# microsoft/AI2BMD

Hardware: NVIDIA H100
Metric: MD steps/sec (higher is better)
Workload: dtype f32

## Files before the change

ai2bmd_b200/csrc/k_edge_tc.cuh:

```cuda
#pragma once
#include "k_edge.cuh"
#include "tc_common.cuh"

namespace vb {

constexpr int TC_TE = 128;
constexpr int TC_STAGES = 2;
constexpr int TC_MAX_STAGES = 3;
constexpr int TC_SLABS = D / tc::SLAB_K;
static_assert((TC_SLABS & (TC_SLABS - 1)) == 0, "tc_slab rotates the slab order with a mask: TC_SLABS must be a power of two");
constexpr int TC_MAXJOBS = 12;
constexpr int TC_LT = D + LDS_PAD;

struct TcJob {
    const float* img;
    int accumulate;
};

struct TcShared {
    alignas(1024) uint8_t ring[TC_STAGES][tc::STAGE_BYTES];
    alignas(16) float tile[TC_TE][TC_LT];
    alignas(16) float abuf[TC_TE][TC_LT];
    EdgeMeta<TC_TE> meta;
    alignas(8) uint64_t b_full[TC_MAX_STAGES];
    uint64_t b_tile;
    uint32_t released[TC_MAX_STAGES];
    const TcJob* jobs;
// ... 77 lines not shown
    __syncwarp();
    if (lane == 0) {
        const uint32_t before = tc::atom_add_acq_rel(&sh.released[k % NS], 1u);
        if (before % TC2_CWARPS == TC2_CWARPS - 1) tc_issue<NS>(sh, k + NS);
    }
}

__device__ __forceinline__ void tc2_tile_to_a(TcShared& sh, int rows) {
    csync();
    for (int idx = threadIdx.x; idx < rows * (D / 4); idx += TC2_CTHREADS) {
        const int r = idx >> 5, c = (idx & 31) * 4;
        st4(&sh.abuf[r][c], ld4(&sh.tile[r][c]));
    }
}

template <int ROWS>
__device__ __forceinline__ void tc2_mma(TcShared& sh, TcRing<ROWS>& ring, float (&acc)[32], int accumulate, int warp, int lane,
                                        int nvalid) {
    constexpr int NS = TcRing<ROWS>::NS;
    csync();
    const int q = warp >> 2, m0 = (q & 1) * 64 + (warp & 3) * 16, g = lane >> 2, t = lane & 3;
    const bool active = (q & 1) * 64 < nvalid;
    if (!accumulate) {
#pragma unroll
        for (int i = 0; i < 32; i++) acc[i] = 0.f;
    }
#pragma unroll 1
    for (int s = 0; s < TC_SLABS; s++) {
        const int k = ring.next + s, stage = k % NS;
        if (active) {
            uint32_t ahi[4][4], alo[4][4];
            const int k0 = tc_slab(s) * tc::SLAB_K + t;
#pragma unroll
            for (int kk = 0; kk < 4; kk++) {
                const int kc = k0 + kk * 8;
                tc::split_tf32(sh.abuf[m0 + g][kc], ahi[kk][0], alo[kk][0]);
                tc::split_tf32(sh.abuf[m0 + g + 8][kc], ahi[kk][1], alo[kk][1]);
                tc::split_tf32(sh.abuf[m0 + g][kc + 4], ahi[kk][2], alo[kk][2]);
                tc::split_tf32(sh.abuf[m0 + g + 8][kc + 4], ahi[kk][3], alo[kk][3]);
            }
            tc::mbar_wait(&sh.b_full[stage], (uint32_t)(k / NS) & 1u);
            const uint32_t bhi = tc::smem_u32(tc_stage_ptr(sh, stage)) + (uint32_t)(q >> 1) * (64 * 128);
            const uint32_t blo = bhi + tc::SLAB_BYTES;
            tc::wgmma_fence();
#pragma unroll
            for (int kk = 0; kk < 4; kk++) {
                const uint64_t dhi = tc::smem_desc_sw128(bhi + kk * 32);
                const uint64_t dlo = tc::smem_desc_sw128(blo + kk * 32);
                tc::mma_m64n64k8_tf32(acc, alo[kk], dhi);
                tc::mma_m64n64k8_tf32(acc, ahi[kk], dlo);
                tc::mma_m64n64k8_tf32(acc, ahi[kk], dhi);
            }
            tc::wgmma_commit();
            tc::wgmma_wait_all();
#pragma unroll
            for (int kk = 0; kk < 4; kk++)
#pragma unroll
                for (int i = 0; i < 4; i++) { tc::reg_fence(ahi[kk][i]); tc::reg_fence(alo[kk][i]); }
#pragma unroll
            for (int i = 0; i < 32; i++) tc::reg_fence(acc[i]);
        } else {
            tc::mbar_wait(&sh.b_full[stage], (uint32_t)(k / NS) & 1u);
        }
        tc2_release<NS>(sh, k, lane);
    }
    ring.next += TC_SLABS;
}

__device__ __forceinline__ void tc2_acc_to_tile(TcShared& sh, const float (&acc)[32], int warp, int lane, int nvalid) {
    const int q = warp >> 2, r = (q & 1) * 64 + (warp & 3) * 16 + (lane >> 2), c = (q >> 1) * 64 + 2 * (lane & 3);
#pragma unroll
    for (int i = 0; i < 8; i++) {
        if (r < nvalid) *reinterpret_cast<float2*>(&sh.tile[r][c + 8 * i]) = make_float2(acc[4 * i], acc[4 * i + 1]);
        if (r + 8 < nvalid) *reinterpret_cast<float2*>(&sh.tile[r + 8][c + 8 * i]) = make_float2(acc[4 * i + 2], acc[4 * i + 3]);
    }
}

template <int ROWS>
__global__ void __launch_bounds__(TC2_THREADS, 1) tc_selftest_kernel(const float* __restrict__ A, const float* __restrict__ img,
                                                                     float* __restrict__ Dout, int reps) {
    extern __shared__ __align__(1024) uint8_t dyn_raw[];
    TcShared& sh = *tc_shared_base(dyn_raw);
    __shared__ TcJob jobs[1];
    if (threadIdx.x == 0) jobs[0] = TcJob{img, 0};
    TcRing<ROWS> ring;
    tc2_setup(sh, ring, jobs, 1, reps);
    const int warp = threadIdx.x >> 5, lane = threadIdx.x & 31;
    float acc[32];
    for (int t = 0; t < reps; t++) {
        for (int idx = threadIdx.x; idx < ROWS * (D / 4); idx += TC2_CTHREADS) {
            const int r = idx >> 5, c = (idx & 31) * 4;
            st4(&sh.tile[r][c], ld4(A + (size_t)r * D + c));
        }
        tc2_tile_to_a(sh, ROWS);
        tc2_mma(sh, ring, acc, 0, warp, lane, ROWS);
        csync();
        tc2_acc_to_tile(sh, acc, warp, lane, ROWS);
        csync();
        for (int idx = threadIdx.x; idx < ROWS * (D / 4); idx += TC2_CTHREADS) {
            const int r = idx >> 5, c = (idx & 31) * 4;
            st4(Dout + (size_t)r * D + c, ld4(&sh.tile[r][c]));
        }
        csync();
    }
}

template <int ROWS>
__global__ void __launch_bounds__(TC2_THREADS, 1) edge_fwd_tc_kernel(const __grid_constant__ EdgeTcArgs a) {
    pdl_entry();
    extern __shared__ __align__(1024) uint8_t dyn_raw[];
    TcShared& sh = *tc_shared_base(dyn_raw);
    const Workspace& ws = a.ws;
    const int l = a.layer;
    const LayerW& lw = a.mw.layer[l];
    const bool upd = (l < L - 1);
    const int J_DK = 0, J_DV = 1, J_F = 2, J_S1 = upd ? 3 : 2, J_S2 = upd ? 4 : 3;
    constexpr int RPW = ROWS / TC2_CWARPS;
    const int warp = threadIdx.x >> 5, lane = threadIdx.x & 31, col = lane * 4;
    const int E = ws.rowptr[ws.N];
    const int trows = min(ROWS, max(16, a.tile_rows));
    const int ntiles_total = (E + trows - 1) / trows;
    const int my_tiles = ((int)blockIdx.x < ntiles_total) ? (ntiles_total - (int)blockIdx.x + (int)gridDim.x - 1) / (int)gridDim.x : 0;
    if (a.tl != nullptr && blockIdx.x == 0 && threadIdx.x == 0) a.tl[0] = (unsigned long long)clock64();
    TcRing<ROWS> ring;
    tc2_setup(sh, ring, a.jobs, a.njobs, my_tiles);
    if (a.tl != nullptr && blockIdx.x == 0 && threadIdx.x == 0) a.tl[1] = (unsigned long long)clock64();

    float acc[32];
    const float* __restrict__ Fin = ws.F[l];
    float* __restrict__ Fout = upd ? ws.F[l + 1] : nullptr;
    const float* __restrict__ QKV = ws.QKV[l];
    const float* __restrict__ VN = ws.VN[l];
// ... 10 lines not shown
        {
            constexpr int RW = ROWS / TC2_CWARPS;
            const int w0 = warp * RW, wn = max(0, min(RW, nvalid - w0));
            if (lane == 0) {
                if (wn > 0) tc::mbar_arrive_expect_tx(&sh.b_tile, (uint32_t)wn * D * 4);
                else tc::mbar_arrive(&sh.b_tile);
            }
            __syncwarp();
            if (lane < wn) tc::tma_load_1d(&sh.abuf[w0 + lane][0], Fin + (size_t)(e0 + w0 + lane) * D, D * 4, &sh.b_tile);
        }
        load_edge_meta<TC_TE, TC2_CTHREADS>(sh.meta, ws, e0, nvalid);
        tc::mbar_wait(&sh.b_tile, tpar);
        csync();
        TC_TL(2);
        float Areg[RPW];
        tc2_mma(sh, ring, acc, a.jobs[J_DK].accumulate, warp, lane, nvalid);
        TC_TL(4);
        tc2_acc_to_tile(sh, acc, warp, lane, nvalid);
        csync();
        {
            TC_TL(5);
            const float4 bb = ldg4(lw.b1 + col);
#pragma unroll
            for (int r = 0; r < RPW; r++) {
                if (r >= rpw) break;
                const int row = r0 + r;
                const float4 qi = ldg4(QKV + (size_t)sh.meta.dst[row] * 3 * D + col);
                const float4 kj = ldg4(QKV + (size_t)sh.meta.src[row] * 3 * D + D + col);
                const float4 P = ld4(&sh.tile[row][col]) + bb;
                const float av = quad_sum(hsum4(qi * kj * silu4(P)));
                Areg[r] = silu_(av) * sh.meta.C[row];
                if ((r < rpw && row < nvalid)) {
                    st4(P1 + (size_t)(e0 + row) * 3 * D + col, P);
                    if ((lane & 3) == 0) ATT[(size_t)(e0 + row) * H + (lane >> 2)] = av;
                }
            }
        }
        TC_TL(6);
        tc2_mma(sh, ring, acc, a.jobs[J_DV].accumulate, warp, lane, nvalid);
        TC_TL(7);
        csync();
        tc2_acc_to_tile(sh, acc, warp, lane, nvalid);
        csync();
        {
            TC_TL(8);
            const float4 bb = ldg4(lw.b1 + D + col);
#pragma unroll
            for (int r = 0; r < RPW; r++) {
                if (r >= rpw) break;
                const int row = r0 + r;
                const float4 vj = ldg4(QKV + (size_t)sh.meta.src[row] * 3 * D + 2 * D + col);
                const float4 P = ld4(&sh.tile[row][col]) + bb;
                st4(&sh.tile[row][col], vj * silu4(P) * Areg[r]);
                if ((r < rpw && row < nvalid)) st4(P1 + (size_t)(e0 + row) * 3 * D + D + col, P);
            }
        }
        csync();
        TC_TL(9);
        {
            const int i_first = sh.meta.dst[0], i_last = sh.meta.dst[nvalid - 1];
            for (int i = i_first + grp; i <= i_last; i += TC2_NGRP) {
                const int q0 = ws.rowptr[i], q1 = ws.rowptr[i + 1];
                const int lo = max(q0, e0) - e0, hi = min(q1, e0 + nvalid) - e0;
                float xa = 0.f;
                for (int r = lo; r < hi; r++) xa += sh.tile[r][cch];
                if (q0 >= e0 && q1 <= e0 + nvalid) ws.XA[(size_t)i * D + cch] = xa;
                else atomicAdd(ws.XA + (size_t)i * D + cch, xa);
            }
        }
        TC_TL(10);
        if (upd) tc2_mma(sh, ring, acc, a.jobs[J_F].accumulate, warp, lane, nvalid);
        tc2_tile_to_a(sh, nvalid);
        TC_TL(11);
        if (upd) {
            csync();
            tc2_acc_to_tile(sh, acc, warp, lane, nvalid);
            csync();
            const float4 bb = ldg4(lw.b1 + 2 * D + col);
#pragma unroll 1
            for (int rb = 0; rb < RPW; rb += 2) {
                if (rb >= rpw) break;
                float4 tir[2][3], ujr[2][3], fin[2];
#pragma unroll
                for (int u = 0; u < 2; u++) {
                    const int row = r0 + rb + u;
                    const size_t i3 = (size_t)sh.meta.dst[row] * 3, j3 = (size_t)sh.meta.src[row] * 3;
                    fin[u] = (rb + u < rpw && row < nvalid) ? ldg4(Fin + (size_t)(e0 + row) * D + col) : f4s(0.f);
#pragma unroll
                    for (int s = 0; s < 3; s++) {
                        tir[u][s] = ldg4(TU + (i3 + s) * 2 * D + col);
                        ujr[u][s] = ldg4(TU + (j3 + s) * 2 * D + D + col);
                    }
                }
#pragma unroll
                for (int u = 0; u < 2; u++) {
                    const int row = r0 + rb + u;
                    const float4 dd = sh.meta.d[row];
                    const float4 Pf = ld4(&sh.tile[row][col]) + bb;
                    const float4 fp = silu4(Pf);
                    const float4 a1 = tir[u][0] * dd.x + tir[u][1] * dd.y + tir[u][2] * dd.z;
                    const float4 a2 = ujr[u][0] * dd.x + ujr[u][1] * dd.y + ujr[u][2] * dd.z;
                    const float4 wdot = (tir[u][0] - a1 * dd.x) * (ujr[u][0] - a2 * dd.x) + (tir[u][1] - a1 * dd.y) * (ujr[u][1] - a2 * dd.y) +
                                        (tir[u][2] - a1 * dd.z) * (ujr[u][2] - a2 * dd.z);
                    if ((rb + u < rpw && row < nvalid)) {
                        st4(P1 + (size_t)(e0 + row) * 3 * D + 2 * D + col, Pf);
                        st4(Fout + (size_t)(e0 + row) * D + col, fin[u] + fp * wdot);
                    }
                }
            }
        }
        TC_TL(12);
        float bnd[2][3] = {{0.f, 0.f, 0.f}, {0.f, 0.f, 0.f}};
        tc2_mma(sh, ring, acc, a.jobs[J_S1].accumulate, warp, lane, nvalid);
        TC_TL(13);
        csync();
        tc2_acc_to_tile(sh, acc, warp, lane, nvalid);
        csync();
        {
            TC_TL(14);
            const float b = __ldg(lw.bs + cch);
            const int i_first = sh.meta.dst[0], i_last = sh.meta.dst[nvalid - 1];
            int nb = 0;
            for (int i = i_first + grp; i <= i_last; i += TC2_NGRP) {
                const int q0 = ws.rowptr[i], q1 = ws.rowptr[i + 1];
                const int lo = max(q0, e0) - e0, hi = min(q1, e0 + nvalid) - e0;
                float v0 = 0.f, v1 = 0.f, v2 = 0.f;
                int r = lo;
                for (; r + 4 <= hi; r += 4) {
                    float g[4][3], s1[4];
#pragma unroll
                    for (int u = 0; u < 4; u++) {
                        const size_t j3 = (size_t)sh.meta.src[r + u] * 3;
                        g[u][0] = __ldg(VN + (j3 + 0) * D + cch); g[u][1] = __ldg(VN + (j3 + 1) * D + cch); g[u][2] = __ldg(VN + (j3 + 2) * D + cch);
                        const float sp = sh.tile[r + u][cch] + b;
                        SP[(size_t)(e0 + r + u) * 2 * D + cch] = sp;
                        s1[u] = silu_(sp);
                    }
#pragma unroll
                    for (int u = 0; u < 4; u++) { v0 += g[u][0] * s1[u]; v1 += g[u][1] * s1[u]; v2 += g[u][2] * s1[u]; }
                }
                for (; r < hi; r++) {
                    const size_t j3 = (size_t)sh.meta.src[r] * 3;
                    const float sp = sh.tile[r][cch] + b;
                    SP[(size_t)(e0 + r) * 2 * D + cch] = sp;
                    const float s1 = silu_(sp);
                    v0 += __ldg(VN + (j3 + 0) * D + cch) * s1;
                    v1 += __ldg(VN + (j3 + 1) * D + cch) * s1;
                    v2 += __ldg(VN + (j3 + 2) * D + cch) * s1;
                }
                if (q0 >= e0 && q1 <= e0 + nvalid) {
                    ws.VA[((size_t)i * 3 + 0) * D + cch] = v0;
                    ws.VA[((size_t)i * 3 + 1) * D + cch] = v1;
                    ws.VA[((size_t)i * 3 + 2) * D + cch] = v2;
                } else if (nb < 2) {
                    bnd[nb][0] = v0; bnd[nb][1] = v1; bnd[nb][2] = v2;
                    nb++;
                }
            }
        }
        TC_TL(15);
        if (threadIdx.x == 0 && it + 1 < my_tiles) {
            const int en = ((int)blockIdx.x + (it + 1) * (int)gridDim.x) * trows;
            tc::tma_prefetch_l2(Fin + (size_t)en * D, (uint32_t)min(trows, E - en) * D * 4);
        }
        tc2_mma(sh, ring, acc, a.jobs[J_S2].accumulate, warp, lane, nvalid);
        TC_TL(16);
        csync();
        tc2_acc_to_tile(sh, acc, warp, lane, nvalid);
        csync();
        {
            TC_TL(17);
            const float b = __ldg(lw.bs + D + cch);
            const int i_first = sh.meta.dst[0], i_last = sh.meta.dst[nvalid - 1];
            int nb = 0;
            for (int i = i_first + grp; i <= i_last; i += TC2_NGRP) {
                const int q0 = ws.rowptr[i], q1 = ws.rowptr[i + 1];
                const int lo = max(q0, e0) - e0, hi = min(q1, e0 + nvalid) - e0;
                float v0 = 0.f, v1 = 0.f, v2 = 0.f;
                for (int r = lo; r < hi; r++) {
                    const float4 de = sh.meta.d[r];
                    const float sp = sh.tile[r][cch] + b;
                    SP[(size_t)(e0 + r) * 2 * D + D + cch] = sp;
                    const float s2 = silu_(sp);
                    v0 += s2 * de.x; v1 += s2 * de.y; v2 += s2 * de.z;
                }
                if (q0 >= e0 && q1 <= e0 + nvalid) {
                    ws.VA[((size_t)i * 3 + 0) * D + cch] += v0;
                    ws.VA[((size_t)i * 3 + 1) * D + cch] += v1;
                    ws.VA[((size_t)i * 3 + 2) * D + cch] += v2;
                } else if (nb < 2) {
                    atomicAdd(ws.VA + ((size_t)i * 3 + 0) * D + cch, bnd[nb][0] + v0);
                    atomicAdd(ws.VA + ((size_t)i * 3 + 1) * D + cch, bnd[nb][1] + v1);
                    atomicAdd(ws.VA + ((size_t)i * 3 + 2) * D + cch, bnd[nb][2] + v2);
                    nb++;
                }
            }
// ... 8 lines not shown

namespace vb {

template <int ROWS>
__global__ void __launch_bounds__(TC2_THREADS, 1) edge_bwd_tc_kernel(const __grid_constant__ EdgeTcArgs a) {
    pdl_entry();
    extern __shared__ __align__(1024) uint8_t dyn_raw[];
    TcShared& sh = *tc_shared_base(dyn_raw);
    const Workspace& ws = a.ws;
    const int l = a.layer;
    const bool upd = (l < L - 1);
    const int J_G3A = 0, J_G3B = 1, J_G4DV = 2, J_G4DK = 3, J_G4F = 4;
    const int J_LAST = upd ? J_G4F : J_G4DK;
    constexpr int RPW = ROWS / TC2_CWARPS;
    constexpr int RB4 = (RPW % 4 == 0) ? 4 : 2;
    const int warp = threadIdx.x >> 5, lane = threadIdx.x & 31, col = lane * 4, hd = lane >> 2;
    const int E = ws.rowptr[ws.N];
    const int trows = min(ROWS, max(16, a.tile_rows));
    const int ntiles_total = (E + trows - 1) / trows;
    const int my_tiles = ((int)blockIdx.x < ntiles_total) ? (ntiles_total - (int)blockIdx.x + (int)gridDim.x - 1) / (int)gridDim.x : 0;
    if (a.tl != nullptr && blockIdx.x == 0 && threadIdx.x == 0) a.tl[0] = (unsigned long long)clock64();
    TcRing<ROWS> ring;
    tc2_setup(sh, ring, a.jobs, a.njobs, my_tiles);
    if (a.tl != nullptr && blockIdx.x == 0 && threadIdx.x == 0) a.tl[1] = (unsigned long long)clock64();

    float acc[32];
    const float* __restrict__ QKV = ws.QKV[l];
    const float* __restrict__ VN = ws.VN[l];
    const float* __restrict__ TU = ws.TU[l];
    const float* __restrict__ P1 = ws.P1[l];
    const float* __restrict__ SP = ws.SP[l];
    const float* __restrict__ ATT = ws.ATT[l];
    const int cch = threadIdx.x & (D - 1), grp = threadIdx.x >> 7;
    for (int it = 0; it < my_tiles; it++) {
        const int e0 = ((int)blockIdx.x + it * (int)gridDim.x) * trows;
        const int nvalid = min(trows, E - e0);
        const int rpw = (nvalid + TC2_CWARPS - 1) / TC2_CWARPS, r0 = warp * rpw;
        load_edge_meta<TC_TE, TC2_CTHREADS>(sh.meta, ws, e0, nvalid);
        csync();
        TC_TL(2);
#pragma unroll 1
        for (int rb = 0; rb < RPW; rb += RB4) {
            if (rb >= rpw) break;
            float4 sp[RB4], gM[RB4][3], vn[RB4][3];
#pragma unroll
            for (int u = 0; u < RB4; u++) {
                const int row = r0 + rb + u;
                const size_t e = (size_t)(e0 + ((rb + u < rpw && row < nvalid) ? row : 0));
                const size_t i3 = (size_t)sh.meta.dst[row] * 3, j3 = (size_t)sh.meta.src[row] * 3;
                sp[u] = ldg4(SP + e * 2 * D + col);
#pragma unroll
                for (int s = 0; s < 3; s++) { gM[u][s] = ldg4(ws.GVEC + (i3 + s) * D + col); vn[u][s] = ldg4(VN + (j3 + s) * D + col); }
            }
#pragma unroll
            for (int u = 0; u < RB4; u++) {
                const int row = r0 + rb + u;
                const bool ok = (rb + u < rpw && row < nvalid);
                const size_t j3 = (size_t)sh.meta.src[row] * 3;
                const float4 s1 = silu4(sp[u]);
                const float4 gs1 = gM[u][0] * vn[u][0] + gM[u][1] * vn[u][1] + gM[u][2] * vn[u][2];
                if (rb + u < rpw) st4(&sh.abuf[row][col], ok ? gs1 * dsilu4(sp[u]) : f4s(0.f));
                if (ok) {
                    red4(ws.GVNMSG + (j3 + 0) * D + col, gM[u][0] * s1);
                    red4(ws.GVNMSG + (j3 + 1) * D + col, gM[u][1] * s1);
                    red4(ws.GVNMSG + (j3 + 2) * D + col, gM[u][2] * s1);
                }
            }
        }
        TC_TL(3);
#pragma unroll 4
        for (int r = 0; r < RPW; r++) {
            if (r >= rpw) break;
            const int row = r0 + r;
            const bool ok = (r < rpw && row < nvalid);
            const size_t e = (size_t)(e0 + (ok ? row : 0));
            const size_t i3 = (size_t)sh.meta.dst[row] * 3;
            const float4 dd = sh.meta.d[row];
            const float4 sp = ldg4(SP + e * 2 * D + D + col);
            const float4 s2 = silu4(sp);
            const float4 gM0 = ldg4(ws.GVEC + (i3 + 0) * D + col), gM1 = ldg4(ws.GVEC + (i3 + 1) * D + col),
                         gM2 = ldg4(ws.GVEC + (i3 + 2) * D + col);
            const float gx_ = warp_sum(hsum4(gM0 * s2)), gy_ = warp_sum(hsum4(gM1 * s2)), gz_ = warp_sum(hsum4(gM2 * s2));
            if (lane == 0) { sh.eacc[row][1] = gx_; sh.eacc[row][2] = gy_; sh.eacc[row][3] = gz_; }
            st4(&sh.tile[row][col], ok ? (gM0 * dd.x + gM1 * dd.y + gM2 * dd.z) * dsilu4(sp) : f4s(0.f));
        }
        TC_TL(5);
        csync();
        tc2_mma(sh, ring, acc, a.jobs[J_G3A].accumulate, warp, lane, nvalid);
        TC_TL(6);
        tc2_tile_to_a(sh, nvalid);
        TC_TL(7);
        tc2_mma(sh, ring, acc, a.jobs[J_G3B].accumulate, warp, lane, nvalid);
        TC_TL(8);
        csync();
        tc2_acc_to_tile(sh, acc, warp, lane, nvalid);
        csync();
        TC_TL(9);
#pragma unroll 1
        for (int rb = 0; rb < RPW; rb += RB4) {
            if (rb >= rpw) break;
            float4 gxa[RB4], vjr[RB4], pdvr[RB4];
            float avr[RB4];
#pragma unroll
            for (int u = 0; u < RB4; u++) {
                const int row = r0 + rb + u;
                const size_t e = (size_t)(e0 + ((rb + u < rpw && row < nvalid) ? row : 0));
                gxa[u] = load_gxa(ws, (size_t)sh.meta.dst[row], col);
                vjr[u] = ldg4(QKV + (size_t)sh.meta.src[row] * 3 * D + 2 * D + col);
                pdvr[u] = ldg4(P1 + e * 3 * D + D + col);
                avr[u] = (rb + u < rpw && row < nvalid) ? __ldg(ATT + e * H + hd) : 0.f;
            }
#pragma unroll
            for (int u = 0; u < RB4; u++) {
                const int row = r0 + rb + u;
                const bool ok = (rb + u < rpw && row < nvalid);
                const size_t j = sh.meta.src[row];
                const float Ce = sh.meta.C[row];
                const float av = avr[u], sa = silu_(av), A = sa * Ce;
                const bool mine = rb + u < rpw;
                const float4 gm = mine ? ld4(&sh.tile[row][col]) + gxa[u] : f4s(0.f);
                const float4 dv = silu4(pdvr[u]);
                if (mine) st4(&sh.abuf[row][col], ok ? gm * vjr[u] * A * dsilu4(pdvr[u]) : f4s(0.f));
                const float gA = quad_sum(hsum4(gm * vjr[u] * dv));
                if (mine && (lane & 3) == 0) sh.gattn[row][hd] = gA * Ce * dsilu_(av);
                const float gc = warp_sum((lane & 3) == 0 ? gA * sa : 0.f);
                if (mine && lane == 0) sh.eacc[row][0] = gc;
                if (ok) red4(ws.GQKV + j * 3 * D + 2 * D + col, gm * dv * A);
            }
// ... 8 lines not shown
            for (int u = 0; u < RB4; u++) {
                const int row = r0 + rb + u;
                const size_t e = (size_t)(e0 + ((rb + u < rpw && row < nvalid) ? row : 0));
                pdkr[u] = ldg4(P1 + e * 3 * D + col);
                qir[u] = ldg4(QKV + (size_t)sh.meta.dst[row] * 3 * D + col);
                kjr[u] = ldg4(QKV + (size_t)sh.meta.src[row] * 3 * D + D + col);
            }
#pragma unroll
            for (int u = 0; u < RB4; u++) {
                const int row = r0 + rb + u;
                const bool ok = (rb + u < rpw && row < nvalid);
                const size_t j = sh.meta.src[row];
                const float4 dk = silu4(pdkr[u]);
                const float gav = sh.gattn[row][hd];
                if (rb + u < rpw) st4(&sh.tile[row][col], ok ? qir[u] * kjr[u] * gav * dsilu4(pdkr[u]) : f4s(0.f));
                if (ok) red4(ws.GQKV + j * 3 * D + D + col, qir[u] * dk * gav);
            }
        }
        TC_TL(12);
        csync();
        tc2_mma(sh, ring, acc, a.jobs[J_G4DV].accumulate, warp, lane, nvalid);
        TC_TL(13);
        tc2_tile_to_a(sh, nvalid);
        TC_TL(14);
        csync();
#pragma unroll 4
        for (int r = 0; r < RPW; r++) {
            if (r >= rpw) break;
            const int row = r0 + r;
            const size_t e = (size_t)(e0 + ((r < rpw && row < nvalid) ? row : 0));
            const float4 dk = silu4(ldg4(P1 + e * 3 * D + col));
            const float4 kj = ldg4(QKV + (size_t)sh.meta.src[row] * 3 * D + D + col);
            st4(&sh.tile[row][col], kj * dk * sh.gattn[row][hd]);
        }
        csync();
        {
            const int i_first = sh.meta.dst[0], i_last = sh.meta.dst[nvalid - 1];
            for (int i = i_first + grp; i <= i_last; i += TC2_NGRP) {
                const int q0 = ws.rowptr[i], q1 = ws.rowptr[i + 1];
                const int lo = max(q0, e0) - e0, hi = min(q1, e0 + nvalid) - e0;
                float gq = 0.f;
                for (int r = lo; r < hi; r++) gq += sh.tile[r][cch];
                if (q0 >= e0 && q1 <= e0 + nvalid) ws.GQKV[(size_t)i * 3 * D + cch] = gq;
                else atomicAdd(ws.GQKV + (size_t)i * 3 * D + cch, gq);
            }
        }
        TC_TL(15);
        if (upd) {
            csync();
#pragma unroll 1
            for (int rb = 0; rb < RPW; rb += 2) {
                if (rb >= rpw) break;
                float4 gfr[2], pfr[2], tir[2][3], ujr[2][3];
#pragma unroll
                for (int u = 0; u < 2; u++) {
                    const int row = r0 + rb + u;
                    const bool ok = (rb + u < rpw && row < nvalid);
                    const size_t e = (size_t)(e0 + (ok ? row : 0));
                    const size_t i3 = (size_t)sh.meta.dst[row] * 3, j3 = (size_t)sh.meta.src[row] * 3;
                    gfr[u] = ok ? ld4(ws.GF + e * D + col) : f4s(0.f);
                    pfr[u] = ldg4(P1 + e * 3 * D + 2 * D + col);
#pragma unroll
                    for (int s = 0; s < 3; s++) {
// ... 6 lines not shown
                    const int row = r0 + rb + u;
                    const bool ok = (rb + u < rpw && row < nvalid);
                    const size_t e = (size_t)(e0 + (ok ? row : 0));
                    const size_t j3 = (size_t)sh.meta.src[row] * 3;
                    const float4 dd = sh.meta.d[row];
                    const float4 gfn = gfr[u], pf = pfr[u];
                    const float4 fp = silu4(pf);
                    const float dv3[3] = {dd.x, dd.y, dd.z};
                    const float4 a1 = tir[u][0] * dd.x + tir[u][1] * dd.y + tir[u][2] * dd.z;
                    const float4 a2 = ujr[u][0] * dd.x + ujr[u][1] * dd.y + ujr[u][2] * dd.z;
                    float4 w1[3], w2[3];
#pragma unroll
                    for (int s = 0; s < 3; s++) { w1[s] = tir[u][s] - a1 * dv3[s]; w2[s] = ujr[u][s] - a2 * dv3[s]; }
                    const float4 wdot = w1[0] * w2[0] + w1[1] * w2[1] + w1[2] * w2[2];
                    const float4 gwd = gfn * fp;
                    if (rb + u < rpw) st4(&sh.tile[row][col], gfn * wdot * dsilu4(pf));
                    const float4 c1 = gwd * (w2[0] * dd.x + w2[1] * dd.y + w2[2] * dd.z);
                    const float4 c2 = gwd * (w1[0] * dd.x + w1[1] * dd.y + w1[2] * dd.z);
                    float gdl[3];
                    float4 gu[3];
#pragma unroll
                    for (int s = 0; s < 3; s++) {
                        const float4 gw1 = gwd * w2[s], gw2 = gwd * w1[s];
                        gu[s] = gw2 - c2 * dv3[s];
                        gdl[s] = warp_sum(hsum4(tir[u][s] * c1 + a1 * gw1 + ujr[u][s] * c2 + a2 * gw2));
                    }
                    if (lane == 0 && rb + u < rpw) { sh.eacc[row][1] -= gdl[0]; sh.eacc[row][2] -= gdl[1]; sh.eacc[row][3] -= gdl[2]; }
                    if (ok) {
                        red4(ws.GTU + (j3 + 0) * 2 * D + D + col, gu[0]);
                        red4(ws.GTU + (j3 + 1) * 2 * D + D + col, gu[1]);
                        red4(ws.GTU + (j3 + 2) * 2 * D + D + col, gu[2]);
                    }
                    (void)e;
                }
            }
            TC_TL(16);
            csync();
            tc2_mma(sh, ring, acc, a.jobs[J_G4DK].accumulate, warp, lane, nvalid);
            TC_TL(17);
            tc2_tile_to_a(sh, nvalid);
            TC_TL(18);
            csync();
#pragma unroll 4
            for (int r = 0; r < RPW; r++) {
                if (r >= rpw) break;
                const int row = r0 + r;
                const bool ok = (r < rpw && row < nvalid);
                const size_t e = (size_t)(e0 + (ok ? row : 0));
                const float4 gfn = ok ? ld4(ws.GF + e * D + col) : f4s(0.f);
                st4(&sh.tile[row][col], gfn * silu4(ldg4(P1 + e * 3 * D + 2 * D + col)));
            }
            csync();
            {
                const int i_first = sh.meta.dst[0], i_last = sh.meta.dst[nvalid - 1];
                for (int i = i_first + grp; i <= i_last; i += TC2_NGRP) {
                    const int q0 = ws.rowptr[i], q1 = ws.rowptr[i + 1];
                    const int lo = max(q0, e0) - e0, hi = min(q1, e0 + nvalid) - e0;
                    float gt0 = 0.f, gt1 = 0.f, gt2 = 0.f;
                    auto term = [&](int r, float u0, float u1, float u2) {
                        const float4 dd = sh.meta.d[r];
                        const float gw = sh.tile[r][cch];
                        const float a2 = u0 * dd.x + u1 * dd.y + u2 * dd.z;
                        const float w20 = u0 - a2 * dd.x, w21 = u1 - a2 * dd.y, w22 = u2 - a2 * dd.z;
                        const float wd = w20 * dd.x + w21 * dd.y + w22 * dd.z;
                        gt0 += gw * (w20 - wd * dd.x);
                        gt1 += gw * (w21 - wd * dd.y);
                        gt2 += gw * (w22 - wd * dd.z);
                    };
                    int r = lo;
                    for (; r + 4 <= hi; r += 4) {
                        float u[4][3];
#pragma unroll
                        for (int q = 0; q < 4; q++) {
                            const size_t j3 = (size_t)sh.meta.src[r + q] * 3;
                            u[q][0] = __ldg(TU + (j3 + 0) * 2 * D + D + cch);
                            u[q][1] = __ldg(TU + (j3 + 1) * 2 * D + D + cch);
// ... 15 lines not shown
                        atomicAdd(ws.GTU + ((size_t)i * 3 + 0) * 2 * D + cch, gt0);
                        atomicAdd(ws.GTU + ((size_t)i * 3 + 1) * 2 * D + cch, gt1);
                        atomicAdd(ws.GTU + ((size_t)i * 3 + 2) * 2 * D + cch, gt2);
                    }
                }
            }
        }
        TC_TL(19);
        if (threadIdx.x < 3 && it + 1 < my_tiles) {
            const int en = ((int)blockIdx.x + (it + 1) * (int)gridDim.x) * trows;
            const uint32_t nn = (uint32_t)min(trows, E - en);
            if (threadIdx.x == 0) tc::tma_prefetch_l2(SP + (size_t)en * 2 * D, nn * 2 * D * 4);
            else if (threadIdx.x == 1) tc::tma_prefetch_l2(P1 + (size_t)en * 3 * D, nn * 3 * D * 4);
            else tc::tma_prefetch_l2(ATT + (size_t)en * H, nn * H * 4);
        }
        tc2_mma(sh, ring, acc, a.jobs[J_LAST].accumulate, warp, lane, nvalid);
        TC_TL(20);
        csync();
        tc2_acc_to_tile(sh, acc, warp, lane, nvalid);
        csync();
        TC_TL(21);
#pragma unroll 4
        for (int r = 0; r < RPW; r++) {
            if (r >= rpw) break;
            const int row = r0 + r;
            if ((r < rpw && row < nvalid)) {
                float* g = ws.GF + (size_t)(e0 + row) * D + col;
                float4 v = ld4(&sh.tile[row][col]);
                if (upd) v = v + ld4(g);
                st4(g, v);
            }
        }
        if (threadIdx.x < nvalid) {
            float* ea = ws.eacc + (size_t)(e0 + threadIdx.x) * 4;
// ... 10 lines not shown
```

ai2bmd_b200/csrc/k_node_tc.cuh:

```cuda
#pragma once
#include "k_edge_tc.cuh"
#include "k_node.cuh"

namespace vb {

enum { NT_OPROJ = 0, NT_PROJ = 1, NT_BWDA = 2, NT_BWDB = 3 };

struct NodeTcArgs {
    int layer;
    ModelW mw;
    Workspace ws;
    int tx, tv;
    int njx, njv;
    int jx, jv;
    TcJob jobs_x[3];
    TcJob jobs_v[5];
    const float* acc_qkv;
    const float* acc_tu;
};

template <int MODE>
__global__ void __launch_bounds__(TC2_THREADS, 1) node_tc_kernel(const __grid_constant__ NodeTcArgs a) {
    pdl_entry();
    extern __shared__ __align__(1024) uint8_t dyn_raw[];
// ... 42 lines not shown
                    } else {
                        const float4 g_vdot = ld4(ws.GX + node * D + col) * ld4(orow + D + col);
                        v = g_vdot * ld4(ws.V123[k] + row * 3 * D + (jj == 0 ? D : 0) + col);
                    }
                }
            } else {
                v = ld4(ws.GO + row * 3 * D + jj * D + col);
            }
            st4(&sh.tile[r][col], v);
        }
    };
    if (!KCHUNKS) {
        load_a(0);
        tc2_tile_to_a(sh, nvalid);
        for (int j = 0; j < nj; j++) {
            tc2_mma(sh, ring, acc, jl[j].accumulate, warp, lane, nvalid);
            csync();
            tc2_acc_to_tile(sh, acc, warp, lane, nvalid);
            csync();
            const int jj = j0 + j;
            for (int r = warp; r < nvalid; r += TC2_CWARPS) {
                const size_t row = (size_t)(row0 + r);
                const float4 v = ld4(&sh.tile[r][col]);
                if (MODE == NT_OPROJ) {
                    st4(ws.O[k - 1] + row * 3 * D + jj * D + col, v + ldg4(a.mw.layer[k - 1].bo + jj * D + col));
                } else {
                    if (is_x) st4(ws.QKV[k] + row * 3 * D + jj * D + col, v + ldg4(a.mw.layer[k].bqkv + jj * D + col));
                    else if (jj < 3) st4(ws.V123[k] + row * 3 * D + jj * D + col, v);
                    else st4(ws.TU[k] + row * 2 * D + (jj - 3) * D + col, v);
                }
            }
        }
    } else {
        for (int j = 0; j < nj; j++) {
            load_a(j0 + j);
            tc2_tile_to_a(sh, nvalid);
            tc2_mma(sh, ring, acc, jl[j].accumulate, warp, lane, nvalid);
        }
        csync();
        tc2_acc_to_tile(sh, acc, warp, lane, nvalid);
        csync();
        for (int r = warp; r < nvalid; r += TC2_CWARPS) {
            const size_t row = (size_t)(row0 + r);
            const float4 v = ld4(&sh.tile[r][col]);
            if (MODE == NT_BWDA) {
                if (is_x) st4(ws.PX + ((size_t)j0 * ws.N + row) * D + col, v);
                else st4(ws.PV + ((size_t)j0 * 3 * ws.N + row) * D + col, v);
            } else {
                st4(ws.GXA + ((size_t)j0 * ws.N + row) * D + col, v);
            }
        }
    }
}

constexpr int NN_WARPS = 8;
// ... 102 lines not shown
```

Before: 1042.

## Use spare tile rows as auxiliary buffers to skip copies and syncs for small edge tiles

```diff
diff --git a/ai2bmd_b200/csrc/k_edge_tc.cuh b/ai2bmd_b200/csrc/k_edge_tc.cuh
--- a/ai2bmd_b200/csrc/k_edge_tc.cuh
+++ b/ai2bmd_b200/csrc/k_edge_tc.cuh
@@ -11,6 +11,7 @@
 static_assert((TC_SLABS & (TC_SLABS - 1)) == 0, "tc_slab rotates the slab order with a mask: TC_SLABS must be a power of two");
 constexpr int TC_MAXJOBS = 12;
 constexpr int TC_LT = D + LDS_PAD;
+typedef float TcRow[TC_LT];
 
 struct TcJob {
     const float* img;
@@ -118,9 +119,11 @@
     }
 }
 
+__device__ __forceinline__ TcRow* tc_aux(TcShared& sh) { return sh.tile + 64; }
+
 template <int ROWS>
-__device__ __forceinline__ void tc2_mma(TcShared& sh, TcRing<ROWS>& ring, float (&acc)[32], int accumulate, int warp, int lane,
-                                        int nvalid) {
+__device__ __forceinline__ void tc2_mma(TcShared& sh, TcRing<ROWS>& ring, const TcRow* A, float (&acc)[32], int accumulate,
+                                        int warp, int lane, int nvalid) {
     constexpr int NS = TcRing<ROWS>::NS;
     csync();
     const int q = warp >> 2, m0 = (q & 1) * 64 + (warp & 3) * 16, g = lane >> 2, t = lane & 3;
@@ -138,10 +141,10 @@
 #pragma unroll
             for (int kk = 0; kk < 4; kk++) {
                 const int kc = k0 + kk * 8;
-                tc::split_tf32(sh.abuf[m0 + g][kc], ahi[kk][0], alo[kk][0]);
-                tc::split_tf32(sh.abuf[m0 + g + 8][kc], ahi[kk][1], alo[kk][1]);
-                tc::split_tf32(sh.abuf[m0 + g][kc + 4], ahi[kk][2], alo[kk][2]);
-                tc::split_tf32(sh.abuf[m0 + g + 8][kc + 4], ahi[kk][3], alo[kk][3]);
+                tc::split_tf32(A[m0 + g][kc], ahi[kk][0], alo[kk][0]);
+                tc::split_tf32(A[m0 + g + 8][kc], ahi[kk][1], alo[kk][1]);
+                tc::split_tf32(A[m0 + g][kc + 4], ahi[kk][2], alo[kk][2]);
+                tc::split_tf32(A[m0 + g + 8][kc + 4], ahi[kk][3], alo[kk][3]);
             }
             tc::mbar_wait(&sh.b_full[stage], (uint32_t)(k / NS) & 1u);
             const uint32_t bhi = tc::smem_u32(tc_stage_ptr(sh, stage)) + (uint32_t)(q >> 1) * (64 * 128);
@@ -171,12 +174,12 @@
     ring.next += TC_SLABS;
 }
 
-__device__ __forceinline__ void tc2_acc_to_tile(TcShared& sh, const float (&acc)[32], int warp, int lane, int nvalid) {
+__device__ __forceinline__ void tc2_acc_to(TcRow* dst, const float (&acc)[32], int warp, int lane, int nvalid) {
     const int q = warp >> 2, r = (q & 1) * 64 + (warp & 3) * 16 + (lane >> 2), c = (q >> 1) * 64 + 2 * (lane & 3);
 #pragma unroll
     for (int i = 0; i < 8; i++) {
-        if (r < nvalid) *reinterpret_cast<float2*>(&sh.tile[r][c + 8 * i]) = make_float2(acc[4 * i], acc[4 * i + 1]);
-        if (r + 8 < nvalid) *reinterpret_cast<float2*>(&sh.tile[r + 8][c + 8 * i]) = make_float2(acc[4 * i + 2], acc[4 * i + 3]);
+        if (r < nvalid) *reinterpret_cast<float2*>(&dst[r][c + 8 * i]) = make_float2(acc[4 * i], acc[4 * i + 1]);
+        if (r + 8 < nvalid) *reinterpret_cast<float2*>(&dst[r + 8][c + 8 * i]) = make_float2(acc[4 * i + 2], acc[4 * i + 3]);
     }
 }
 
@@ -197,9 +200,9 @@
             st4(&sh.tile[r][c], ld4(A + (size_t)r * D + c));
         }
         tc2_tile_to_a(sh, ROWS);
-        tc2_mma(sh, ring, acc, 0, warp, lane, ROWS);
-        csync();
-        tc2_acc_to_tile(sh, acc, warp, lane, ROWS);
+        tc2_mma(sh, ring, sh.abuf, acc, 0, warp, lane, ROWS);
+        csync();
+        tc2_acc_to(sh.tile, acc, warp, lane, ROWS);
         csync();
         for (int idx = threadIdx.x; idx < ROWS * (D / 4); idx += TC2_CTHREADS) {
             const int r = idx >> 5, c = (idx & 31) * 4;
@@ -220,6 +223,7 @@
     const bool upd = (l < L - 1);
     const int J_DK = 0, J_DV = 1, J_F = 2, J_S1 = upd ? 3 : 2, J_S2 = upd ? 4 : 3;
     constexpr int RPW = ROWS / TC2_CWARPS;
+    constexpr bool SMALL = ROWS <= 64;
     const int warp = threadIdx.x >> 5, lane = threadIdx.x & 31, col = lane * 4;
     const int E = ws.rowptr[ws.N];
     const int trows = min(ROWS, max(16, a.tile_rows));
@@ -260,9 +264,9 @@
         csync();
         TC_TL(2);
         float Areg[RPW];
-        tc2_mma(sh, ring, acc, a.jobs[J_DK].accumulate, warp, lane, nvalid);
+        tc2_mma(sh, ring, sh.abuf, acc, a.jobs[J_DK].accumulate, warp, lane, nvalid);
         TC_TL(4);
-        tc2_acc_to_tile(sh, acc, warp, lane, nvalid);
+        tc2_acc_to(sh.tile, acc, warp, lane, nvalid);
         csync();
         {
             TC_TL(5);
@@ -283,10 +287,10 @@
             }
         }
         TC_TL(6);
-        tc2_mma(sh, ring, acc, a.jobs[J_DV].accumulate, warp, lane, nvalid);
+        tc2_mma(sh, ring, sh.abuf, acc, a.jobs[J_DV].accumulate, warp, lane, nvalid);
         TC_TL(7);
         csync();
-        tc2_acc_to_tile(sh, acc, warp, lane, nvalid);
+        tc2_acc_to(sh.tile, acc, warp, lane, nvalid);
         csync();
         {
             TC_TL(8);
@@ -315,12 +319,13 @@
             }
         }
         TC_TL(10);
-        if (upd) tc2_mma(sh, ring, acc, a.jobs[J_F].accumulate, warp, lane, nvalid);
-        tc2_tile_to_a(sh, nvalid);
+        if (upd) tc2_mma(sh, ring, sh.abuf, acc, a.jobs[J_F].accumulate, warp, lane, nvalid);
+        if constexpr (!SMALL) tc2_tile_to_a(sh, nvalid);
         TC_TL(11);
         if (upd) {
-            csync();
-            tc2_acc_to_tile(sh, acc, warp, lane, nvalid);
+            TcRow* const pfb = SMALL ? tc_aux(sh) : sh.tile;
+            if constexpr (!SMALL) csync();
+            tc2_acc_to(pfb, acc, warp, lane, nvalid);
             csync();
             const float4 bb = ldg4(lw.b1 + 2 * D + col);
 #pragma unroll 1
@@ -331,7 +336,8 @@
                 for (int u = 0; u < 2; u++) {
                     const int row = r0 + rb + u;
                     const size_t i3 = (size_t)sh.meta.dst[row] * 3, j3 = (size_t)sh.meta.src[row] * 3;
-                    fin[u] = (rb + u < rpw && row < nvalid) ? ldg4(Fin + (size_t)(e0 + row) * D + col) : f4s(0.f);
+                    if (rb + u < rpw && row < nvalid) fin[u] = SMALL ? ld4(&sh.abuf[row][col]) : ldg4(Fin + (size_t)(e0 + row) * D + col);
+                    else fin[u] = f4s(0.f);
 #pragma unroll
                     for (int s = 0; s < 3; s++) {
                         tir[u][s] = ldg4(TU + (i3 + s) * 2 * D + col);
@@ -342,7 +348,7 @@
                 for (int u = 0; u < 2; u++) {
                     const int row = r0 + rb + u;
                     const float4 dd = sh.meta.d[row];
-                    const float4 Pf = ld4(&sh.tile[row][col]) + bb;
+                    const float4 Pf = ld4(&pfb[row][col]) + bb;
                     const float4 fp = silu4(Pf);
                     const float4 a1 = tir[u][0] * dd.x + tir[u][1] * dd.y + tir[u][2] * dd.z;
                     const float4 a2 = ujr[u][0] * dd.x + ujr[u][1] * dd.y + ujr[u][2] * dd.z;
@@ -357,10 +363,11 @@
         }
         TC_TL(12);
         float bnd[2][3] = {{0.f, 0.f, 0.f}, {0.f, 0.f, 0.f}};
-        tc2_mma(sh, ring, acc, a.jobs[J_S1].accumulate, warp, lane, nvalid);
+        TcRow* const s1b = SMALL ? tc_aux(sh) : sh.tile;
+        tc2_mma(sh, ring, SMALL ? sh.tile : sh.abuf, acc, a.jobs[J_S1].accumulate, warp, lane, nvalid);
         TC_TL(13);
-        csync();
-        tc2_acc_to_tile(sh, acc, warp, lane, nvalid);
+        if constexpr (!SMALL) csync();
+        tc2_acc_to(s1b, acc, warp, lane, nvalid);
         csync();
         {
             TC_TL(14);
@@ -378,7 +385,7 @@
                     for (int u = 0; u < 4; u++) {
                         const size_t j3 = (size_t)sh.meta.src[r + u] * 3;
                         g[u][0] = __ldg(VN + (j3 + 0) * D + cch); g[u][1] = __ldg(VN + (j3 + 1) * D + cch); g[u][2] = __ldg(VN + (j3 + 2) * D + cch);
-                        const float sp = sh.tile[r + u][cch] + b;
+                        const float sp = s1b[r + u][cch] + b;
                         SP[(size_t)(e0 + r + u) * 2 * D + cch] = sp;
                         s1[u] = silu_(sp);
                     }
@@ -387,7 +394,7 @@
                 }
                 for (; r < hi; r++) {
                     const size_t j3 = (size_t)sh.meta.src[r] * 3;
-                    const float sp = sh.tile[r][cch] + b;
+                    const float sp = s1b[r][cch] + b;
                     SP[(size_t)(e0 + r) * 2 * D + cch] = sp;
                     const float s1 = silu_(sp);
                     v0 += __ldg(VN + (j3 + 0) * D + cch) * s1;
@@ -409,10 +416,11 @@
             const int en = ((int)blockIdx.x + (it + 1) * (int)gridDim.x) * trows;
             tc::tma_prefetch_l2(Fin + (size_t)en * D, (uint32_t)min(trows, E - en) * D * 4);
         }
-        tc2_mma(sh, ring, acc, a.jobs[J_S2].accumulate, warp, lane, nvalid);
+        TcRow* const s2b = SMALL ? sh.abuf : sh.tile;
+        tc2_mma(sh, ring, SMALL ? sh.tile : sh.abuf, acc, a.jobs[J_S2].accumulate, warp, lane, nvalid);
         TC_TL(16);
-        csync();
-        tc2_acc_to_tile(sh, acc, warp, lane, nvalid);
+        if constexpr (!SMALL) csync();
+        tc2_acc_to(s2b, acc, warp, lane, nvalid);
         csync();
         {
             TC_TL(17);
@@ -425,7 +433,7 @@
                 float v0 = 0.f, v1 = 0.f, v2 = 0.f;
                 for (int r = lo; r < hi; r++) {
                     const float4 de = sh.meta.d[r];
-                    const float sp = sh.tile[r][cch] + b;
+                    const float sp = s2b[r][cch] + b;
                     SP[(size_t)(e0 + r) * 2 * D + D + cch] = sp;
                     const float s2 = silu_(sp);
                     v0 += s2 * de.x; v1 += s2 * de.y; v2 += s2 * de.z;
@@ -464,6 +472,8 @@
     const int J_LAST = upd ? J_G4F : J_G4DK;
     constexpr int RPW = ROWS / TC2_CWARPS;
     constexpr int RB4 = (RPW % 4 == 0) ? 4 : 2;
+    constexpr bool SMALL = ROWS <= 64;
+    constexpr int RBM = SMALL ? 2 : RB4;
     const int warp = threadIdx.x >> 5, lane = threadIdx.x & 31, col = lane * 4, hd = lane >> 2;
     const int E = ws.rowptr[ws.N];
     const int trows = min(ROWS, max(16, a.tile_rows));
@@ -489,70 +499,111 @@
         load_edge_meta<TC_TE, TC2_CTHREADS>(sh.meta, ws, e0, nvalid);
         csync();
         TC_TL(2);
+        if constexpr (SMALL) {
 #pragma unroll 1
-        for (int rb = 0; rb < RPW; rb += RB4) {
-            if (rb >= rpw) break;
-            float4 sp[RB4], gM[RB4][3], vn[RB4][3];
-#pragma unroll
-            for (int u = 0; u < RB4; u++) {
-                const int row = r0 + rb + u;
-                const size_t e = (size_t)(e0 + ((rb + u < rpw && row < nvalid) ? row : 0));
-                const size_t i3 = (size_t)sh.meta.dst[row] * 3, j3 = (size_t)sh.meta.src[row] * 3;
-                sp[u] = ldg4(SP + e * 2 * D + col);
-#pragma unroll
-                for (int s = 0; s < 3; s++) { gM[u][s] = ldg4(ws.GVEC + (i3 + s) * D + col); vn[u][s] = ldg4(VN + (j3 + s) * D + col); }
-            }
-#pragma unroll
-            for (int u = 0; u < RB4; u++) {
-                const int row = r0 + rb + u;
-                const bool ok = (rb + u < rpw && row < nvalid);
-                const size_t j3 = (size_t)sh.meta.src[row] * 3;
-                const float4 s1 = silu4(sp[u]);
-                const float4 gs1 = gM[u][0] * vn[u][0] + gM[u][1] * vn[u][1] + gM[u][2] * vn[u][2];
-                if (rb + u < rpw) st4(&sh.abuf[row][col], ok ? gs1 * dsilu4(sp[u]) : f4s(0.f));
-                if (ok) {
-                    red4(ws.GVNMSG + (j3 + 0) * D + col, gM[u][0] * s1);
-                    red4(ws.GVNMSG + (j3 + 1) * D + col, gM[u][1] * s1);
-                    red4(ws.GVNMSG + (j3 + 2) * D + col, gM[u][2] * s1);
-                }
-            }
-        }
-        TC_TL(3);
+            for (int rb = 0; rb < RPW; rb += RB4) {
+                if (rb >= rpw) break;
+                float4 sp[RB4][2], gM[RB4][3], vn[RB4][3];
+#pragma unroll
+                for (int u = 0; u < RB4; u++) {
+                    const int row = r0 + rb + u;
+                    const size_t e = (size_t)(e0 + ((rb + u < rpw && row < nvalid) ? row : 0));
+                    const size_t i3 = (size_t)sh.meta.dst[row] * 3, j3 = (size_t)sh.meta.src[row] * 3;
+                    sp[u][0] = ldg4(SP + e * 2 * D + col);
+                    sp[u][1] = ldg4(SP + e * 2 * D + D + col);
+#pragma unroll
+                    for (int s = 0; s < 3; s++) { gM[u][s] = ldg4(ws.GVEC + (i3 + s) * D + col); vn[u][s] = ldg4(VN + (j3 + s) * D + col); }
+                }
+#pragma unroll
+                for (int u = 0; u < RB4; u++) {
+                    const int row = r0 + rb + u;
+                    const bool mine = rb + u < rpw, ok = (mine && row < nvalid);
+                    const size_t j3 = (size_t)sh.meta.src[row] * 3;
+                    const float4 dd = sh.meta.d[row];
+                    const float4 s1 = silu4(sp[u][0]), s2 = silu4(sp[u][1]);
+                    const float4 gs1 = gM[u][0] * vn[u][0] + gM[u][1] * vn[u][1] + gM[u][2] * vn[u][2];
+                    const float gx_ = warp_sum(hsum4(gM[u][0] * s2)), gy_ = warp_sum(hsum4(gM[u][1] * s2)), gz_ = warp_sum(hsum4(gM[u][2] * s2));
+                    if (mine) {
+                        st4(&sh.abuf[row][col], ok ? gs1 * dsilu4(sp[u][0]) : f4s(0.f));
+                        st4(&sh.tile[row][col], ok ? (gM[u][0] * dd.x + gM[u][1] * dd.y + gM[u][2] * dd.z) * dsilu4(sp[u][1]) : f4s(0.f));
+                        if (lane == 0) { sh.eacc[row][1] = gx_; sh.eacc[row][2] = gy_; sh.eacc[row][3] = gz_; }
+                    }
+                    if (ok) {
+                        red4(ws.GVNMSG + (j3 + 0) * D + col, gM[u][0] * s1);
+                        red4(ws.GVNMSG + (j3 + 1) * D + col, gM[u][1] * s1);
+                        red4(ws.GVNMSG + (j3 + 2) * D + col, gM[u][2] * s1);
+                    }
+                }
+            }
+            TC_TL(3);
+        } else {
+#pragma unroll 1
+            for (int rb = 0; rb < RPW; rb += RB4) {
+                if (rb >= rpw) break;
+                float4 sp[RB4], gM[RB4][3], vn[RB4][3];
+#pragma unroll
+                for (int u = 0; u < RB4; u++) {
+                    const int row = r0 + rb + u;
+                    const size_t e = (size_t)(e0 + ((rb + u < rpw && row < nvalid) ? row : 0));
+                    const size_t i3 = (size_t)sh.meta.dst[row] * 3, j3 = (size_t)sh.meta.src[row] * 3;
+                    sp[u] = ldg4(SP + e * 2 * D + col);
+#pragma unroll
+                    for (int s = 0; s < 3; s++) { gM[u][s] = ldg4(ws.GVEC + (i3 + s) * D + col); vn[u][s] = ldg4(VN + (j3 + s) * D + col); }
+                }
+#pragma unroll
+                for (int u = 0; u < RB4; u++) {
+                    const int row = r0 + rb + u;
+                    const bool ok = (rb + u < rpw && row < nvalid);
+                    const size_t j3 = (size_t)sh.meta.src[row] * 3;
+                    const float4 s1 = silu4(sp[u]);
+                    const float4 gs1 = gM[u][0] * vn[u][0] + gM[u][1] * vn[u][1] + gM[u][2] * vn[u][2];
+                    if (rb + u < rpw) st4(&sh.abuf[row][col], ok ? gs1 * dsilu4(sp[u]) : f4s(0.f));
+                    if (ok) {
+                        red4(ws.GVNMSG + (j3 + 0) * D + col, gM[u][0] * s1);
+                        red4(ws.GVNMSG + (j3 + 1) * D + col, gM[u][1] * s1);
+                        red4(ws.GVNMSG + (j3 + 2) * D + col, gM[u][2] * s1);
+                    }
+                }
+            }
+            TC_TL(3);
 #pragma unroll 4
-        for (int r = 0; r < RPW; r++) {
-            if (r >= rpw) break;
-            const int row = r0 + r;
-            const bool ok = (r < rpw && row < nvalid);
-            const size_t e = (size_t)(e0 + (ok ? row : 0));
-            const size_t i3 = (size_t)sh.meta.dst[row] * 3;
-            const float4 dd = sh.meta.d[row];
-            const float4 sp = ldg4(SP + e * 2 * D + D + col);
-            const float4 s2 = silu4(sp);
-            const float4 gM0 = ldg4(ws.GVEC + (i3 + 0) * D + col), gM1 = ldg4(ws.GVEC + (i3 + 1) * D + col),
-                         gM2 = ldg4(ws.GVEC + (i3 + 2) * D + col);
-            const float gx_ = warp_sum(hsum4(gM0 * s2)), gy_ = warp_sum(hsum4(gM1 * s2)), gz_ = warp_sum(hsum4(gM2 * s2));
-            if (lane == 0) { sh.eacc[row][1] = gx_; sh.eacc[row][2] = gy_; sh.eacc[row][3] = gz_; }
-            st4(&sh.tile[row][col], ok ? (gM0 * dd.x + gM1 * dd.y + gM2 * dd.z) * dsilu4(sp) : f4s(0.f));
-        }
-        TC_TL(5);
-        csync();
-        tc2_mma(sh, ring, acc, a.jobs[J_G3A].accumulate, warp, lane, nvalid);
+            for (int r = 0; r < RPW; r++) {
+                if (r >= rpw) break;
+                const int row = r0 + r;
+                const bool ok = (r < rpw && row < nvalid);
+                const size_t e = (size_t)(e0 + (ok ? row : 0));
+                const size_t i3 = (size_t)sh.meta.dst[row] * 3;
+                const float4 dd = sh.meta.d[row];
+                const float4 sp = ldg4(SP + e * 2 * D + D + col);
+                const float4 s2 = silu4(sp);
+                const float4 gM0 = ldg4(ws.GVEC + (i3 + 0) * D + col), gM1 = ldg4(ws.GVEC + (i3 + 1) * D + col),
+                             gM2 = ldg4(ws.GVEC + (i3 + 2) * D + col);
+                const float gx_ = warp_sum(hsum4(gM0 * s2)), gy_ = warp_sum(hsum4(gM1 * s2)), gz_ = warp_sum(hsum4(gM2 * s2));
+                if (lane == 0) { sh.eacc[row][1] = gx_; sh.eacc[row][2] = gy_; sh.eacc[row][3] = gz_; }
+                st4(&sh.tile[row][col], ok ? (gM0 * dd.x + gM1 * dd.y + gM2 * dd.z) * dsilu4(sp) : f4s(0.f));
+            }
+            TC_TL(5);
+        }
+        csync();
+        tc2_mma(sh, ring, sh.abuf, acc, a.jobs[J_G3A].accumulate, warp, lane, nvalid);
         TC_TL(6);
-        tc2_tile_to_a(sh, nvalid);
-        TC_TL(7);
-        tc2_mma(sh, ring, acc, a.jobs[J_G3B].accumulate, warp, lane, nvalid);
+        if constexpr (!SMALL) {
+            tc2_tile_to_a(sh, nvalid);
+            TC_TL(7);
+        }
+        tc2_mma(sh, ring, SMALL ? sh.tile : sh.abuf, acc, a.jobs[J_G3B].accumulate, warp, lane, nvalid);
         TC_TL(8);
         csync();
-        tc2_acc_to_tile(sh, acc, warp, lane, nvalid);
+        tc2_acc_to(sh.tile, acc, warp, lane, nvalid);
         csync();
         TC_TL(9);
 #pragma unroll 1
-        for (int rb = 0; rb < RPW; rb += RB4) {
+        for (int rb = 0; rb < RPW; rb += RBM) {
             if (rb >= rpw) break;
-            float4 gxa[RB4], vjr[RB4], pdvr[RB4];
-            float avr[RB4];
-#pragma unroll
-            for (int u = 0; u < RB4; u++) {
+            float4 gxa[RBM], vjr[RBM], pdvr[RBM];
+            float avr[RBM];
+#pragma unroll
+            for (int u = 0; u < RBM; u++) {
                 const int row = r0 + rb + u;
                 const size_t e = (size_t)(e0 + ((rb + u < rpw && row < nvalid) ? row : 0));
                 gxa[u] = load_gxa(ws, (size_t)sh.meta.dst[row], col);
@@ -561,7 +612,7 @@
                 avr[u] = (rb + u < rpw && row < nvalid) ? __ldg(ATT + e * H + hd) : 0.f;
             }
 #pragma unroll
-            for (int u = 0; u < RB4; u++) {
+            for (int u = 0; u < RBM; u++) {
                 const int row = r0 + rb + u;
                 const bool ok = (rb + u < rpw && row < nvalid);
                 const size_t j = sh.meta.src[row];
@@ -600,39 +651,44 @@
                 const float4 dk = silu4(pdkr[u]);
                 const float gav = sh.gattn[row][hd];
                 if (rb + u < rpw) st4(&sh.tile[row][col], ok ? qir[u] * kjr[u] * gav * dsilu4(pdkr[u]) : f4s(0.f));
+                if (SMALL && rb + u < rpw) st4(&tc_aux(sh)[row][col], kjr[u] * dk * gav);
                 if (ok) red4(ws.GQKV + j * 3 * D + D + col, qir[u] * dk * gav);
             }
         }
         TC_TL(12);
         csync();
-        tc2_mma(sh, ring, acc, a.jobs[J_G4DV].accumulate, warp, lane, nvalid);
+        tc2_mma(sh, ring, sh.abuf, acc, a.jobs[J_G4DV].accumulate, warp, lane, nvalid);
         TC_TL(13);
-        tc2_tile_to_a(sh, nvalid);
-        TC_TL(14);
-        csync();
+        if constexpr (!SMALL) {
+            tc2_tile_to_a(sh, nvalid);
+            TC_TL(14);
+            csync();
 #pragma unroll 4
-        for (int r = 0; r < RPW; r++) {
-            if (r >= rpw) break;
-            const int row = r0 + r;
-            const size_t e = (size_t)(e0 + ((r < rpw && row < nvalid) ? row : 0));
-            const float4 dk = silu4(ldg4(P1 + e * 3 * D + col));
-            const float4 kj = ldg4(QKV + (size_t)sh.meta.src[row] * 3 * D + D + col);
-            st4(&sh.tile[row][col], kj * dk * sh.gattn[row][hd]);
-        }
-        csync();
+            for (int r = 0; r < RPW; r++) {
+                if (r >= rpw) break;
+                const int row = r0 + r;
+                const size_t e = (size_t)(e0 + ((r < rpw && row < nvalid) ? row : 0));
+                const float4 dk = silu4(ldg4(P1 + e * 3 * D + col));
+                const float4 kj = ldg4(QKV + (size_t)sh.meta.src[row] * 3 * D + D + col);
+                st4(&sh.tile[row][col], kj * dk * sh.gattn[row][hd]);
+            }
+            csync();
+        }
         {
+            const TcRow* const gqb = SMALL ? tc_aux(sh) : sh.tile;
             const int i_first = sh.meta.dst[0], i_last = sh.meta.dst[nvalid - 1];
             for (int i = i_first + grp; i <= i_last; i += TC2_NGRP) {
                 const int q0 = ws.rowptr[i], q1 = ws.rowptr[i + 1];
                 const int lo = max(q0, e0) - e0, hi = min(q1, e0 + nvalid) - e0;
                 float gq = 0.f;
-                for (int r = lo; r < hi; r++) gq += sh.tile[r][cch];
+                for (int r = lo; r < hi; r++) gq += gqb[r][cch];
                 if (q0 >= e0 && q1 <= e0 + nvalid) ws.GQKV[(size_t)i * 3 * D + cch] = gq;
                 else atomicAdd(ws.GQKV + (size_t)i * 3 * D + cch, gq);
             }
         }
         TC_TL(15);
         if (upd) {
+            TcRow* const gpfb = SMALL ? sh.abuf : sh.tile;
             csync();
 #pragma unroll 1
             for (int rb = 0; rb < RPW; rb += 2) {
@@ -669,7 +725,10 @@
                     for (int s = 0; s < 3; s++) { w1[s] = tir[u][s] - a1 * dv3[s]; w2[s] = ujr[u][s] - a2 * dv3[s]; }
                     const float4 wdot = w1[0] * w2[0] + w1[1] * w2[1] + w1[2] * w2[2];
                     const float4 gwd = gfn * fp;
-                    if (rb + u < rpw) st4(&sh.tile[row][col], gfn * wdot * dsilu4(pf));
+                    if (rb + u < rpw) {
+                        st4(&gpfb[row][col], gfn * wdot * dsilu4(pf));
+                        if (SMALL) st4(&tc_aux(sh)[row][col], gwd);
+                    }
                     const float4 c1 = gwd * (w2[0] * dd.x + w2[1] * dd.y + w2[2] * dd.z);
                     const float4 c2 = gwd * (w1[0] * dd.x + w1[1] * dd.y + w1[2] * dd.z);
                     float gdl[3];
@@ -691,22 +750,25 @@
             }
             TC_TL(16);
             csync();
-            tc2_mma(sh, ring, acc, a.jobs[J_G4DK].accumulate, warp, lane, nvalid);
+            tc2_mma(sh, ring, SMALL ? sh.tile : sh.abuf, acc, a.jobs[J_G4DK].accumulate, warp, lane, nvalid);
             TC_TL(17);
-            tc2_tile_to_a(sh, nvalid);
-            TC_TL(18);
-            csync();
+            if constexpr (!SMALL) {
+                tc2_tile_to_a(sh, nvalid);
+                TC_TL(18);
+                csync();
 #pragma unroll 4
-            for (int r = 0; r < RPW; r++) {
-                if (r >= rpw) break;
-                const int row = r0 + r;
-                const bool ok = (r < rpw && row < nvalid);
-                const size_t e = (size_t)(e0 + (ok ? row : 0));
-                const float4 gfn = ok ? ld4(ws.GF + e * D + col) : f4s(0.f);
-                st4(&sh.tile[row][col], gfn * silu4(ldg4(P1 + e * 3 * D + 2 * D + col)));
-            }
-            csync();
+                for (int r = 0; r < RPW; r++) {
+                    if (r >= rpw) break;
+                    const int row = r0 + r;
+                    const bool ok = (r < rpw && row < nvalid);
+                    const size_t e = (size_t)(e0 + (ok ? row : 0));
+                    const float4 gfn = ok ? ld4(ws.GF + e * D + col) : f4s(0.f);
+                    st4(&sh.tile[row][col], gfn * silu4(ldg4(P1 + e * 3 * D + 2 * D + col)));
+                }
+                csync();
+            }
             {
+                const TcRow* const gwb = SMALL ? tc_aux(sh) : sh.tile;
                 const int i_first = sh.meta.dst[0], i_last = sh.meta.dst[nvalid - 1];
                 for (int i = i_first + grp; i <= i_last; i += TC2_NGRP) {
                     const int q0 = ws.rowptr[i], q1 = ws.rowptr[i + 1];
@@ -714,7 +776,7 @@
                     float gt0 = 0.f, gt1 = 0.f, gt2 = 0.f;
                     auto term = [&](int r, float u0, float u1, float u2) {
                         const float4 dd = sh.meta.d[r];
-                        const float gw = sh.tile[r][cch];
+                        const float gw = gwb[r][cch];
                         const float a2 = u0 * dd.x + u1 * dd.y + u2 * dd.z;
                         const float w20 = u0 - a2 * dd.x, w21 = u1 - a2 * dd.y, w22 = u2 - a2 * dd.z;
                         const float wd = w20 * dd.x + w21 * dd.y + w22 * dd.z;
@@ -760,10 +822,10 @@
             else if (threadIdx.x == 1) tc::tma_prefetch_l2(P1 + (size_t)en * 3 * D, nn * 3 * D * 4);
             else tc::tma_prefetch_l2(ATT + (size_t)en * H, nn * H * 4);
         }
-        tc2_mma(sh, ring, acc, a.jobs[J_LAST].accumulate, warp, lane, nvalid);
+        tc2_mma(sh, ring, (SMALL && !upd) ? sh.tile : sh.abuf, acc, a.jobs[J_LAST].accumulate, warp, lane, nvalid);
         TC_TL(20);
-        csync();
-        tc2_acc_to_tile(sh, acc, warp, lane, nvalid);
+        if (!SMALL || !upd) csync();
+        tc2_acc_to(sh.tile, acc, warp, lane, nvalid);
         csync();
         TC_TL(21);
 #pragma unroll 4
diff --git a/ai2bmd_b200/csrc/k_node_tc.cuh b/ai2bmd_b200/csrc/k_node_tc.cuh
--- a/ai2bmd_b200/csrc/k_node_tc.cuh
+++ b/ai2bmd_b200/csrc/k_node_tc.cuh
@@ -80,9 +80,9 @@
         load_a(0);
         tc2_tile_to_a(sh, nvalid);
         for (int j = 0; j < nj; j++) {
-            tc2_mma(sh, ring, acc, jl[j].accumulate, warp, lane, nvalid);
+            tc2_mma(sh, ring, sh.abuf, acc, jl[j].accumulate, warp, lane, nvalid);
             csync();
-            tc2_acc_to_tile(sh, acc, warp, lane, nvalid);
+            tc2_acc_to(sh.tile, acc, warp, lane, nvalid);
             csync();
             const int jj = j0 + j;
             for (int r = warp; r < nvalid; r += TC2_CWARPS) {
@@ -101,10 +101,10 @@
         for (int j = 0; j < nj; j++) {
             load_a(j0 + j);
             tc2_tile_to_a(sh, nvalid);
-            tc2_mma(sh, ring, acc, jl[j].accumulate, warp, lane, nvalid);
+            tc2_mma(sh, ring, sh.abuf, acc, jl[j].accumulate, warp, lane, nvalid);
         }
         csync();
-        tc2_acc_to_tile(sh, acc, warp, lane, nvalid);
+        tc2_acc_to(sh.tile, acc, warp, lane, nvalid);
         csync();
         for (int r = warp; r < nvalid; r += TC2_CWARPS) {
             const size_t row = (size_t)(row0 + r);
```

After: 1119 (median of 6 runs). +7.3%, better.
